# jmhb0/view_neti

Hardware: AMD Instinct MI355X
Metric: TI train steps/sec (SD-1.5 512^2 bs=4 per GPU) (higher is better)
Workload: dtype f16; 1 GPU; learnable_mode 0, sd15 shapes, 512x512 fp16, bs=4/GPU, grad_accum 1, full train step (VAE+16xCLIP+UNet fwd/bwd+AdamW); global_batch=4, parallelism=dp1, rccl_ranks=1, hipgraph=True

## Files before the change

### include/vneti.h

```cpp
#ifndef VNETI_H
#define VNETI_H
#include <stddef.h>
#include <stdint.h>

#ifdef __cplusplus
extern "C" {
#endif

#define VNETI_ABI_VERSION 1

int vneti_version(void);
int vneti_precision(void);
int vneti_last_error(char* buf, size_t n);

typedef struct vneti_gemm_desc {
  const void* A;
  const void* B;
  void* C;
  long long lda, ldb, ldc;
  int M, N, K;
  int batch;
  long long strideA, strideB, strideC;
  const float* bias;
  const void* rowadd;
  long long ld_rowadd;
  int rows_per_group;
  const void* resid;
  long long ldr;
  float alpha;
  int act;
  int out_f32;
  int conv_mode;
  int Hi, Wi, Ci, Ho, Wo, stride, pad_t, pad_l, ups;
  long long ldx;
  int tile_hint;
  void* workspace;
  long long workspace_bytes;
  int split_k;
  const void* gate_src;
  long long ld_gate;
  int gate_act;
  void* C2;
  long long ldc2;
  int act2;
  void* gn_sums;
  int gn_hw, gn_cpg, gn_groups, gn_slots;
  int geglu;
  int conv_korder;
} vneti_gemm_desc;

int vneti_gemm_f16(const vneti_gemm_desc* d, void* stream);
int vneti_gemm_select_tile(int M, int N, int batch);
int vneti_gemm_select_split(int M, int N, int K, int batch, int tile_hint, long long workspace_bytes);

int vneti_im2col3x3_small(const void* x, int x_is_f32, long long sb, long long sc, long long sy,
                          long long sx, void* out, int Bn, int C, int Hi, int Wi, int Ho, int Wo,
                          int stride, int pad_t, int pad_l, void* stream);

int vneti_conv3x3_in(const void* x, int x_is_f32, long long sb, long long sc, long long sy, long long sx,
                     const void* w_packed, const float* bias, void* out, long long ldo, int Bn, int C, int H, int W,
                     int Co, void* gn_sums, int gn_groups, int gn_slots, void* stream);

int vneti_transpose_f16(const void* in, long long ld_in, long long stride_in, void* out,
                        long long ld_out, long long stride_out, int rows, int cols, int batch,
                        void* stream);
#define VNETI_TRANSPOSE_MAX 4
typedef struct vneti_transpose_desc {
  const void* inp;
  long long ld_in, stride_in;
  void* out;
  long long ld_out, stride_out;
  int rows, cols, batch, _pad;
} vneti_transpose_desc;
int vneti_transpose_f16_multi(const vneti_transpose_desc* descs, int n, void* stream);

long long vneti_groupnorm_ws_floats(int Bn, int HW, int C, int G);
int vneti_groupnorm_fwd(const void* x, long long ldx, void* y, long long ldy, const float* gamma,
                        const float* beta, float* mean, float* rstd, float* ws, int Bn, int HW,
                        int C, int G, float eps, int silu, void* stream);
int vneti_groupnorm_fwd_sums(const void* x, long long ldx, void* y, long long ldy, const float* gamma,
                             const float* beta, const void* sums, int slots, float* mean, float* rstd,
                             int Bn, int HW, int C, int G, float eps, int silu, void* stream);
int vneti_groupnorm_fwd_2l(const void* x, long long ldx, void* y, long long ldy, const float* gamma,
                           const float* beta, void* sums, int slots, float* mean, float* rstd, int Bn, int HW,
// ... 181 lines not shown
```

### view_neti_amd/csrc/gemm8.hip

```cpp
#include <type_traits>

#include "common.h"
#include "gemm_args.h"

namespace {

constexpr int BM = 256, NT = 512;
constexpr int HALF_BYTES = 128 * 128;
constexpr int GN_IMG = 5;

#define VN_WAIT_VM(n) asm volatile("s_waitcnt vmcnt(" #n ")" ::: "memory")
#define VN_WAIT_LGKM0() asm volatile("s_waitcnt lgkmcnt(0)" ::: "memory")

template <int BN, int EPI, bool CONV, bool HALO = false>
__global__ __launch_bounds__(NT) void gemm8_kernel(GemmArgs g) {
  static_assert(BN == 256 || BN == 128, "tile width");
  static_assert(!HALO || (BN == 128 && CONV), "the halo-patch loop exists for the 256x128 convolution tile");
  constexpr int PATCH_STRIDE = 41 * 1024;
  constexpr bool H42 = HALO && BN == 128;
  constexpr int NJB = BN / 128;
  constexpr int HB_BYTES = (BN / 2) * 128;
  constexpr int HB_DMA = BN / 128;
  constexpr int NBUF = BN == 256 ? 2 : 3;
  constexpr int BUF_BYTES = 2 * HALF_BYTES + 2 * HB_BYTES;
  constexpr int CS_LD = BN + 8;
  constexpr int CS_BYTES = BM * CS_LD * 2;
  constexpr int LOOP_BYTES = HALO ? 2 * PATCH_STRIDE + 3 * 2 * HB_BYTES : NBUF * BUF_BYTES;
  constexpr int LDS_BYTES = CS_BYTES > LOOP_BYTES ? CS_BYTES : LOOP_BYTES;
  constexpr int GN_NG = BN / 4 + 2;
  const half_t* const e_gate = EPI == 2 ? g.gate_src : nullptr;
  half_t* const e_C2 = EPI == 2 ? g.C2 : nullptr;
  const int e_geglu = EPI == 2 ? g.geglu : 0;
  const int e_act = EPI == 2 ? g.act : 0;
  float* const e_gn_sums = EPI >= 1 ? g.gn_sums : nullptr;
  const half_t* const e_rowadd = EPI >= 1 ? g.rowadd : nullptr;
  const int e_conv = CONV ? g.conv_mode : 0;
  constexpr int GN_BYTES = EPI == 0 ? 0 : GN_IMG * GN_NG * 4 * 8;
  __shared__ __attribute__((aligned(16))) char smem[LDS_BYTES + GN_BYTES];

  const int tid = threadIdx.x;
  const int lane = tid & 63;
  const int wave = __builtin_amdgcn_readfirstlane(tid >> 6);
  const int wr = wave >> 2, wc = wave & 3;

  int nblk = g.tiles_m * g.tiles_n;
  int bid = blockIdx.x;
  {
    int q = nblk >> 3, r = nblk & 7, xcd = bid & 7, idx = bid >> 3;
    bid = (xcd < r ? xcd * (q + 1) : r * (q + 1) + (xcd - r) * q) + idx;
  }
  const int tile_m = bid / g.tiles_n;
  const int tile_n = bid - tile_m * g.tiles_n;
  const int m0 = tile_m * BM;
  const int n0 = tile_n * BN;
  const int bz = blockIdx.y;
  const int kz = blockIdx.z;
  int hb = 0, hty = 0, htx = 0, row0 = m0;
  if constexpr (HALO) {
    const int tpr = g.Wo >> 4, tpi = (g.Ho >> 4) * tpr;
    hb = tile_m / tpi;
    const int rem = tile_m - hb * tpi;
    hty = rem / tpr;
    htx = rem - hty * tpr;
    row0 = (hb * g.Ho + hty * 16) * g.Wo + htx * 16;
  }
  auto rowmem = [&](const int r) { return HALO ? row0 + (r >> 4) * g.Wo + (r & 15) : m0 + r; };

  const half_t* Ab = g.A + (long long)bz * g.strideA;
  const half_t* Bb = g.B + (long long)bz * g.strideB;
  const __amdgpu_buffer_rsrc_t rsA = vn_make_rsrc(Ab, g.a_bytes);
  const __amdgpu_buffer_rsrc_t rsB = vn_make_rsrc(Bb, g.b_bytes);

  const int lrow = tid >> 3;
  const int gchunk = (tid & 7) ^ ((lrow >> 1) & 7);
  const float rcp_hw = CONV ? 1.0f / (float)(g.Ho * g.Wo) : 0.f, rcp_wo = CONV ? 1.0f / (float)g.Wo : 0.f;
  int a_base[4];
  uint32_t a_mask[4];
#pragma unroll
  for (int r = 0; r < (HALO ? 0 : 4); ++r) {
// ... 719 lines not shown
      const vn_u64* src = gacc + 4 * i;
      if ((src[0] | src[1] | src[2] | src[3]) == 0) continue;
      const int img = gn_img0 + i / GN_NG, grp = gn_g0t + i % GN_NG;
      vn_u64* dst = reinterpret_cast<vn_u64*>(e_gn_sums) + (((long long)img * g.gn_slots + slot) * g.gn_G + grp) * 4;
#pragma unroll
      for (int w = 0; w < 4; ++w) atomicAdd(dst + w, src[w]);
    }
  }
}

inline int epilogue_level8(const GemmArgs& g) {
  if (g.gate_src || g.C2 || g.geglu || g.act) return 2;
  return (g.gn_sums || g.rowadd) ? 1 : 0;
}

}

int vneti_launch_gemm8(void* gemm_args, int bn, int halo, hipStream_t st) {
  GemmArgs& g = *reinterpret_cast<GemmArgs*>(gemm_args);
  if (g.out_f32 || (g.conv_mode && (g.ups || (g.conv_mode == 2 && g.stride == 2))) ||
      (g.M >= (1 << 24) && (g.conv_mode || g.rowadd || g.gn_sums)))
    return VNETI_EUNSUP;
  if (halo && (bn != 128 || g.conv_mode < 1 || g.conv_mode > 2 || g.stride != 1 || g.pad_t != 1 || g.pad_l != 1 || g.Hi != g.Ho ||
               g.Wi != g.Wo || (g.Ho & 15) || (g.Wo & 15) || (g.Ci & 63) || g.K != 9 * g.Ci || !g.korder ||
               g.batch != 1 || g.M != (g.M / (g.Ho * g.Wo)) * g.Ho * g.Wo))
    return VNETI_EUNSUP;
  if (halo && g.ksplit > 1) {
    const int nchunk = g.Ci / 64, cps = cdiv(nchunk, g.ksplit);
    g.kt_per_split = 9 * cps;
    g.ksplit = cdiv(nchunk, cps);
  }
  g.tiles_m = cdiv(g.M, BM);
  g.tiles_n = cdiv(g.N, bn);
  const dim3 grid(g.tiles_m * g.tiles_n, g.batch, g.ksplit), block(NT);
  const int epi = epilogue_level8(g);
#define VN_GO(E, C)                                                                        \
  do {                                                                                     \
    if (bn == 256) hipLaunchKernelGGL((gemm8_kernel<256, E, C>), grid, block, 0, st, g);   \
    else hipLaunchKernelGGL((gemm8_kernel<128, E, C>), grid, block, 0, st, g);             \
  } while (0)
#define VN_GO_HALO(E) hipLaunchKernelGGL((gemm8_kernel<128, E, true, true>), grid, block, 0, st, g)
  if (halo) {
    if (epi == 2) VN_GO_HALO(2); else if (epi == 1) VN_GO_HALO(1); else VN_GO_HALO(0);
  } else if (g.conv_mode) {
    if (epi == 2) VN_GO(2, true); else if (epi == 1) VN_GO(1, true); else VN_GO(0, true);
  } else {
    if (epi == 2) VN_GO(2, false); else if (epi == 1) VN_GO(1, false); else VN_GO(0, false);
  }
#undef VN_GO
#undef VN_GO_HALO
  return vneti_check_launch("gemm8_kernel");
}
```

### view_neti_amd/csrc/gemm_args.h

```cpp
#pragma once
#include "common.h"

namespace {

struct GemmArgs {
  const half_t* A;
  const half_t* B;
  void* C;
  const float* bias;
  const half_t* rowadd;
  const void* resid;
  float* ws;
  const half_t* gate_src;
  half_t* C2;
  long long ld_gate, ldc2;
  int gate_act, act2;
  float* gn_sums;
  int gn_hw, gn_cpg, gn_G, gn_slots;
  int geglu;
  long long lda, ldb, ldc, ld_rowadd, ldr;
  long long strideA, strideB, strideC;
  uint32_t a_bytes, b_bytes;
  int M, N, K;
  int rows_per_group;
  float alpha;
  int act;
  int out_f32;
  int batch, ksplit, kt_per_split;
  int conv_mode;
  int Hi, Wi, Ci, Ho, Wo, stride, pad_t, pad_l, ups;
  int ldx2;
  int korder;
  int tiles_m, tiles_n;
};

__device__ __forceinline__ float apply_act(float v, int act) {
  switch (act) {
    case 1: return vn_silu(v);
    case 2: return vn_quick_gelu(v);
    case 3: return vn_gelu_erf(v);
    default: return v;
  }
}
__device__ __forceinline__ float act_grad(float f, int act) {
  if (act == 2) {
    float s = vn_sigmoid(1.702f * f);
    return s * (1.f + 1.702f * f * (1.f - s));
  } else if (act == 3) {
    return vn_gelu_erf_grad(f);
  }
  float s = vn_sigmoid(f);
  return s * (1.f + f * (1.f - s));
}

__device__ __forceinline__ int lds_off(int row, int chunk) {
  return row * 128 + ((chunk ^ ((row >> 1) & 7)) << 4);
}

__device__ __forceinline__ void dma16(__amdgpu_buffer_rsrc_t rs, char* lds_dst, uint32_t off) {
#if defined(__HIP_DEVICE_COMPILE__)
  __builtin_amdgcn_raw_ptr_buffer_load_lds(rs, (__attribute__((address_space(3))) void*)lds_dst, 16, off, 0, 0, 0);
#else
  (void)rs; (void)lds_dst; (void)off;
#endif
}

}

int vneti_launch_gemm8(void* gemm_args, int bn, int halo, hipStream_t st);
```

### view_neti_amd/csrc/gemm_conv.hip

```cpp
#include "common.h"
#include "gemm_args.h"
#include "../../include/vneti.h"

namespace {

template <int BM, int BN, int WM, int WN, bool F32OUT, bool DMA, int NSTG = 2, int EPI = 2, bool CONV = true>
__global__ __launch_bounds__((BM / WM) * (BN / WN) * 64) void gemm_kernel(
    const half_t* pA, const half_t* pB, uint32_t p_a_bytes, uint32_t p_b_bytes, int p_lda, int p_ldb, int pM, int pN, int pK,
    int p_tiles_m, int p_tiles_n, int p_split_conv , const GemmArgs gfull) {
  GemmArgs g = gfull;
  g.A = pA;
  g.B = pB;
  g.a_bytes = p_a_bytes;
  g.b_bytes = p_b_bytes;
  g.lda = p_lda;
  g.ldb = p_ldb;
  g.M = pM;
  g.N = pN;
  g.K = pK;
  g.tiles_m = p_tiles_m;
  g.tiles_n = p_tiles_n;
  g.kt_per_split = p_split_conv & 0xffff;
  g.ksplit = (p_split_conv >> 16) & 0xff;
  g.conv_mode = p_split_conv >> 24;
  static_assert(NSTG == 2 || ((NSTG == 3 || NSTG == 4) && DMA), "the LDS rings are LDS-DMA only");
  const half_t* const e_gate = EPI == 2 ? g.gate_src : nullptr;
  half_t* const e_C2 = EPI == 2 ? g.C2 : nullptr;
  const int e_geglu = EPI == 2 ? g.geglu : 0;
  const int e_act = EPI == 2 ? g.act : 0;
  float* const e_gn_sums = EPI >= 1 ? g.gn_sums : nullptr;
  const half_t* const e_rowadd = EPI >= 1 ? g.rowadd : nullptr;
  const int e_conv = CONV ? g.conv_mode : 0;
  constexpr int NWM = BM / WM, NWN = BN / WN;
  constexpr int NT = NWM * NWN * 64;
  constexpr int RSTEP = NT / 8;
  constexpr int A_IT = BM / RSTEP, B_IT = BN / RSTEP;
  constexpr int STAGE_BYTES = (BM + BN) * 128;
  constexpr int CS_LD = F32OUT ? (BN + 4) : (BN + 8);
  constexpr int CS_BYTES = BM * CS_LD * (F32OUT ? 4 : 2);
  constexpr int LDS_BYTES = (NSTG * STAGE_BYTES > CS_BYTES) ? NSTG * STAGE_BYTES : CS_BYTES;
  constexpr int GN_IMG = 5, GN_NG = BN / 4 + 2;
  constexpr int GN_BYTES = (F32OUT || EPI == 0) ? 0 : GN_IMG * GN_NG * 4 * 8;
  __shared__ __attribute__((aligned(16))) char smem[LDS_BYTES + GN_BYTES];

  const int tid = threadIdx.x;
  const int lane = tid & 63;
  const int wave = __builtin_amdgcn_readfirstlane(tid >> 6);
  const int wm0 = (wave / NWN) * WM;
  const int wn0 = (wave % NWN) * WN;

  int nblk = g.tiles_m * g.tiles_n;
  int bid = blockIdx.x;
  {
    int q = nblk >> 3, r = nblk & 7, xcd = bid & 7, idx = bid >> 3;
    bid = (xcd < r ? xcd * (q + 1) : r * (q + 1) + (xcd - r) * q) + idx;
  }
  const int tile_m = bid / g.tiles_n;
  const int tile_n = bid - tile_m * g.tiles_n;
  const int m0 = tile_m * BM;
  const int n0 = tile_n * BN;
  const int bz = blockIdx.y;
  const int kz = blockIdx.z;

  const half_t* Ab = g.A + (long long)bz * g.strideA;
  const half_t* Bb = g.B + (long long)bz * g.strideB;
  __amdgpu_buffer_rsrc_t rsA = vn_make_rsrc(Ab, g.a_bytes);
  __amdgpu_buffer_rsrc_t rsB = vn_make_rsrc(Bb, g.b_bytes);

  const int lrow = tid >> 3;
  const int gchunk = DMA ? ((tid & 7) ^ ((lrow >> 1) & 7)) : (tid & 7);

  const float rcp_hw = CONV ? __builtin_amdgcn_rcpf((float)(g.Ho * g.Wo)) : 0.f, rcp_wo = CONV ? __builtin_amdgcn_rcpf((float)g.Wo) : 0.f;
  int a_off[A_IT];
  int a_py[A_IT], a_px[A_IT], a_bh[A_IT];
#pragma unroll
  for (int i = 0; i < A_IT; ++i) {
    int m = m0 + lrow + RSTEP * i;
    bool ok = m < g.M;
    if (e_conv == 0) {
      a_off[i] = ok ? (int)((long long)m * g.lda * 2) + gchunk * 16 : -1;
      a_py[i] = a_px[i] = a_bh[i] = 0;
    } else {
      int rem, ox;
      const int b = vn_divmod(m, g.Ho * g.Wo, rcp_hw, rem);
      const int oy = vn_divmod(rem, g.Wo, rcp_wo, ox);
// ... 535 lines not shown
  for (int z = 0; z < g.ksplit; ++z) {
    const float* p = p0 + z * zstride;
    for (int e = 0; e < ne; ++e) v[e] += p[e];
  }
  for (int e = 0; e < ne; ++e) {
    float x = v[e] * g.alpha;
    if (g.bias) x += g.bias[c + e];
    x = apply_act(x, g.act);
    if (g.out_f32) {
      if (g.resid) x += reinterpret_cast<const float*>(g.resid)[(long long)bz * g.strideC + (long long)m * g.ldr + c + e];
      reinterpret_cast<float*>(g.C)[(long long)bz * g.strideC + (long long)m * g.ldc + c + e] = x;
    } else {
      x = (float)(half_t)x;
      if (g.rowadd) x = (float)(half_t)(x + (float)g.rowadd[(long long)(m / g.rows_per_group) * g.ld_rowadd + c + e]);
      if (g.resid)
        x = (float)(half_t)(x + (float)reinterpret_cast<const half_t*>(g.resid)[(long long)bz * g.strideC + (long long)m * g.ldr + c + e]);
      if (g.gate_src) x = (float)(half_t)(x * act_grad((float)g.gate_src[(long long)m * g.ld_gate + c + e], g.gate_act));
      reinterpret_cast<half_t*>(g.C)[(long long)bz * g.strideC + (long long)m * g.ldc + c + e] = (half_t)x;
      if (g.C2) g.C2[(long long)m * g.ldc2 + c + e] = (half_t)apply_act((float)(half_t)x, g.act2);
    }
  }
}

inline int epilogue_level(const GemmArgs& g) {
  if (g.gate_src || g.C2 || g.geglu || g.act) return 2;
  return (g.gn_sums || g.rowadd) ? 1 : 0;
}

template <int BM, int BN, int WM, int WN, bool F32OUT, bool DMA, int NSTG>
void launch_variant(const GemmArgs& g, dim3 grid, hipStream_t st) {
  const dim3 block((BM / WM) * (BN / WN) * 64);
#define VN_GO(E, C)                                                                                                        \
  hipLaunchKernelGGL((gemm_kernel<BM, BN, WM, WN, F32OUT, DMA, NSTG, E, C>), grid, block, 0, st, g.A, g.B, g.a_bytes, g.b_bytes, \
                     (int)g.lda, (int)g.ldb, g.M, g.N, g.K, g.tiles_m, g.tiles_n, g.kt_per_split | (g.ksplit << 16) | (g.conv_mode << 24), g)
  if constexpr (F32OUT) {
    if (g.conv_mode) { if (g.act) VN_GO(2, true); else VN_GO(0, true); }
    else { if (g.act) VN_GO(2, false); else VN_GO(0, false); }
  } else {
    const int epi = epilogue_level(g);
    if (g.conv_mode) { if (epi == 2) VN_GO(2, true); else if (epi == 1) VN_GO(1, true); else VN_GO(0, true); }
    else { if (epi == 2) VN_GO(2, false); else if (epi == 1) VN_GO(1, false); else VN_GO(0, false); }
  }
#undef VN_GO
}

inline void launch_reduce(const GemmArgs& g, hipStream_t st) {
  if (g.ksplit > 1) {
    long long total = (long long)g.batch * g.M * ((g.N + 3) / 4);
    hipLaunchKernelGGL(splitk_reduce_kernel, dim3((unsigned)cdivl(total, 256)), dim3(256), 0, st, g.ws, g.C, g.bias, g.resid,
                       g.rowadd, g.M, g.N, g.batch, g.ksplit, (int)g.ldc, (int)g.ldr, g);
  }
}

template <int BM, int BN, int WM, int WN, bool DMA>
int launch_cfg(GemmArgs& g, bool f32out, hipStream_t st) {
  g.tiles_m = cdiv(g.M, BM);
  g.tiles_n = cdiv(g.N, BN);
  dim3 grid(g.tiles_m * g.tiles_n, g.batch, g.ksplit);
  if (f32out) launch_variant<BM, BN, WM, WN, true, DMA, 2>(g, grid, st);
  else launch_variant<BM, BN, WM, WN, false, DMA, 2>(g, grid, st);
  launch_reduce(g, st);
  return vneti_check_launch("gemm_kernel");
}

template <int BM, int BN, int WM, int WN, int NSTG = 3>
int launch_cfg_ring(GemmArgs& g, bool f32out, hipStream_t st) {
  g.tiles_m = cdiv(g.M, BM);
  g.tiles_n = cdiv(g.N, BN);
  dim3 grid(g.tiles_m * g.tiles_n, g.batch, g.ksplit);
  if (f32out) launch_variant<BM, BN, WM, WN, true, true, NSTG>(g, grid, st);
  else launch_variant<BM, BN, WM, WN, false, true, NSTG>(g, grid, st);
  launch_reduce(g, st);
  return vneti_check_launch("gemm_kernel");
}

template <int BM, int BN, int WM, int WN, bool DMA>
int launch_cfg_f16(GemmArgs& g, hipStream_t st) {
  g.tiles_m = cdiv(g.M, BM);
  g.tiles_n = cdiv(g.N, BN);
  dim3 grid(g.tiles_m * g.tiles_n, g.batch, g.ksplit);
  launch_variant<BM, BN, WM, WN, false, DMA, 2>(g, grid, st);
  launch_reduce(g, st);
  return vneti_check_launch("gemm_kernel");
}

struct TileDims {
  int bm, bn;
};
constexpr int kMaxTile = 18;
constexpr TileDims kTiles[kMaxTile + 1] = {{0, 0},     {128, 128}, {128, 64},  {64, 64},  {256, 128}, {256, 256}, {256, 128}, {256, 128},
                                          {256, 128}, {128, 128}, {128, 128}, {128, 64},  {64, 64},   {128, 128}, {128, 64},  {64, 64},
                                          {256, 256}, {256, 128}, {256, 128}};

int select_tile(int M, int N, int batch) {
  long long t256 = (long long)cdiv(M, 256) * cdiv(N, 128) * batch;
  long long t128 = (long long)cdiv(M, 128) * cdiv(N, 128) * batch;
  long long t12864 = (long long)cdiv(M, 128) * cdiv(N, 64) * batch;
  if (N <= 64) return (M >= 2048) ? 2 : 3;
  (void)t256;
  if (t128 >= 384) return 1;
  if (t12864 >= 384) return 2;
  return 3;
}

int select_ksplit(int M, int N, int K, int batch, int tile, long long ws_floats) {
  if (ws_floats <= 0) return 1;
  const int nk = K / 64;
  long long tiles = (long long)cdiv(M, kTiles[tile].bm) * cdiv(N, kTiles[tile].bn) * batch;
  if (tiles >= 256 || nk < 16) return 1;
  int s = (int)(512 / tiles);
  if (s > nk / 8) s = nk / 8;
  if (s > 16) s = 16;
  while (s > 1 && (long long)s * batch * M * N > ws_floats) --s;
  return s < 2 ? 1 : s;
}

}

extern "C" int vneti_gemm_select_tile(int M, int N, int batch) { return select_tile(M, N, batch > 0 ? batch : 1); }

extern "C" int vneti_gemm_select_split(int M, int N, int K, int batch, int tile_hint, long long workspace_bytes) {
  if (batch <= 0) batch = 1;
  int cfg = tile_hint >= 100 ? tile_hint - 100 : tile_hint;
  if (cfg == 0) cfg = select_tile(M, N, batch);
  if (cfg < 1 || cfg > kMaxTile || K % 64 != 0) return -1;
  int ks = select_ksplit(M, N, K, batch, cfg, workspace_bytes / 4);
  const int nk = K / 64;
  if (ks > nk) ks = nk;
  if (ks < 1) ks = 1;
  return cdiv(nk, cdiv(nk, ks));
}

extern "C" int vneti_gemm_f16(const vneti_gemm_desc* d, void* stream) {
  VN_REQUIRE(d != nullptr, "gemm: null descriptor");
  VN_REQUIRE(d->A && d->B && d->C, "gemm: null operand pointer");
  VN_REQUIRE(d->M > 0 && d->N > 0 && d->K > 0, "gemm: bad shape M=%d N=%d K=%d", d->M, d->N, d->K);
  VN_REQUIRE(d->K % 64 == 0, "gemm: K=%d must be a multiple of 64", d->K);
  VN_REQUIRE(d->ldb % 8 == 0, "gemm: ldb=%lld must be a multiple of 8", d->ldb);
  int batch = d->batch > 0 ? d->batch : 1;
  GemmArgs g;
  memset(&g, 0, sizeof(g));
  g.A = (const half_t*)d->A;
  g.B = (const half_t*)d->B;
  g.C = d->C;
  g.bias = d->bias;
  g.rowadd = (const half_t*)d->rowadd;
  g.resid = d->resid;
  g.gate_src = (const half_t*)d->gate_src;
  g.ld_gate = d->ld_gate;
  g.gate_act = d->gate_act;
  g.C2 = (half_t*)d->C2;
  g.ldc2 = d->ldc2;
  g.act2 = d->act2;
  g.gn_sums = (float*)d->gn_sums;
  g.gn_hw = d->gn_hw;
  g.gn_cpg = d->gn_cpg;
  g.gn_G = d->gn_groups;
  g.gn_slots = d->gn_slots;
  g.geglu = d->geglu;
  g.lda = d->lda;
  g.ldb = d->ldb;
  g.ldc = d->ldc;
  g.ld_rowadd = d->ld_rowadd;
  g.ldr = d->ldr;
  g.strideA = d->strideA;
  g.strideB = d->strideB;
  g.strideC = d->strideC;
  g.M = d->M;
  g.N = d->N;
  g.K = d->K;
  g.batch = batch;
  g.rows_per_group = d->rows_per_group > 0 ? d->rows_per_group : 1;
  g.alpha = d->alpha;
  g.act = d->act;
  g.out_f32 = d->out_f32 ? 1 : 0;
  g.conv_mode = d->conv_mode;
  long long a_bytes;
  if (d->conv_mode == 0) {
    VN_REQUIRE(d->lda % 8 == 0, "gemm: lda=%lld must be a multiple of 8", d->lda);
    a_bytes = ((long long)(d->M - 1) * d->lda + d->K) * 2;
  } else {
    VN_REQUIRE(d->conv_mode == 1 || d->conv_mode == 2, "gemm: bad conv_mode %d", d->conv_mode);
    VN_REQUIRE(d->Ci > 0 && d->Ci % 64 == 0, "conv: Ci=%d must be a multiple of 64", d->Ci);
    VN_REQUIRE(d->K == 9 * d->Ci, "conv: K=%d must equal 9*Ci=%d", d->K, 9 * d->Ci);
    VN_REQUIRE(d->stride == 1 || d->stride == 2, "conv: stride %d unsupported", d->stride);
    VN_REQUIRE(d->Ho > 0 && d->Wo > 0 && d->M % (d->Ho * d->Wo) == 0, "conv: M=%d not a multiple of Ho*Wo", d->M);
    VN_REQUIRE(d->ldx % 8 == 0, "conv: ldx must be a multiple of 8");
    VN_REQUIRE(!(d->ups && d->conv_mode != 1), "conv: fused upsample only in forward gather mode");
    VN_REQUIRE(!(d->ups && d->stride != 1), "conv: fused upsample needs stride 1");
    g.Hi = d->Hi;
    g.Wi = d->Wi;
    g.Ci = d->Ci;
    g.Ho = d->Ho;
    g.Wo = d->Wo;
    g.stride = d->stride;
    g.pad_t = d->pad_t;
    g.pad_l = d->pad_l;
    g.ups = d->ups;
    g.ldx2 = (int)(d->ldx * 2);
    VN_REQUIRE(!d->conv_korder || d->Ci % 64 == 0, "conv: conv_korder=1 needs Ci=%d to be a multiple of 64", d->Ci);
    g.korder = d->conv_korder ? 1 : 0;
    long long nb = d->M / (d->Ho * d->Wo);
    a_bytes = nb * d->Hi * d->Wi * d->ldx * 2;
  }
  long long b_bytes = ((long long)(d->N - 1) * d->ldb + d->K) * 2;
  VN_REQUIRE(a_bytes < 0x7fffffffLL && b_bytes < 0x7fffffffLL, "gemm: operand larger than 2 GiB");
  g.a_bytes = (uint32_t)a_bytes;
  g.b_bytes = (uint32_t)b_bytes;
  if (!d->out_f32) {
// ... 105 lines not shown
```

### view_neti_amd/engine/schedule.py

```python
from __future__ import annotations

from functools import partial
from typing import Dict, List

import torch

from .. import lib, ops, packing


class T:

    __slots__ = ("v", "g", "gw", "rows", "cols", "children", "need_grad", "producer")

    def __init__(self, v, g=None, need_grad=True):
        self.v = v
        self.g = g
        self.gw = False
        self.rows, self.cols = v.shape
        self.children: List["T"] = []
        self.need_grad = need_grad
        self.producer = None


def rup(x, m):
# ... 411 lines not shown


def _timing_switches(dev, reps):
    import os
    cold = None if os.environ.get("VNETI_AUTOTUNE_HOT") else torch.empty(160 * 2 ** 20, dtype=torch.float32, device=dev)
    return (cold, reps, int(os.environ.get("VNETI_AUTOTUNE_REPS", "9")),
            bool(int(os.environ.get("VNETI_AUTOTUNE_WARM_A", "1"))))


def _time_call(call, act, cold, reps, cold_reps, warm_a):
    call()
    call()

    def timed(n):
        s, e = torch.cuda.Event(enable_timing=True), torch.cuda.Event(enable_timing=True)
        s.record()
        for _ in range(n):
            call()
        e.record()
        e.synchronize()
        return s.elapsed_time(e)

    if cold is None:
        return timed(reps)
    ts = []
    for _ in range(cold_reps):
        cold.fill_(0)
        if warm_a:
            act.add_(0)
        ts.append(timed(1))
    return sorted(ts)[len(ts) // 2]


def picks_to_json(cache: Dict) -> Dict:
    return {repr(k): [int(x) for x in v] for k, v in cache.items()}


def picks_from_json(data: Dict) -> Dict:
    import ast
    return {ast.literal_eval(k): tuple(int(x) for x in v) for k, v in data.items()}


def export_picks() -> Dict:
    from ..roofline import kernel_tree_sha
    return {"kernel_tree_sha": kernel_tree_sha(), "picks": picks_to_json(Schedule._tile_cache)}


def preload_picks(data: Dict) -> bool:
    from ..roofline import kernel_tree_sha
    if data.get("kernel_tree_sha") != kernel_tree_sha():
        return False
    Schedule._tile_cache.update(picks_from_json(data["picks"]))
    return True
```

### view_neti_amd/engine/step.py

```python
from __future__ import annotations

from functools import partial
from typing import Dict, List, Optional

import torch

from .. import ops
from .. import sd_config as sc
from .graphs import capture_graphs
from .text import MapperState, TextEngine
from .unet import UNetEngine
from .vae import VAEEncoderEngine


def alphas_cumprod(cfg: sc.DDPMConfig) -> torch.Tensor:
    betas = torch.linspace(cfg.beta_start ** 0.5, cfg.beta_end ** 0.5, cfg.num_train_timesteps,
                           dtype=torch.float32) ** 2
    return torch.cumprod(1.0 - betas, dim=0)


class TrainStepEngine:
    def __init__(self, cfg: sc.SDConfig, unet_w: Dict, vae_w: Dict, clip_w: Dict, batch: int, height: int,
                 width: int, mapper_object: Dict[str, torch.Tensor], w_enc_object: torch.Tensor,
                 norm_scale_object: Optional[float], alpha_object: float = 0.2,
# ... 61 lines not shown
        mo = MapperState(self.params[:n_all_obj],
                         w_enc_object.to(device).float().contiguous() if legacy_pe_object is None else None,
                         norm_scale_object, alpha_object, hidden=hidden_object, enc_dim=enc_dim_object,
                         unconstrained=unconstrained_object,
                         nested_dropout_prob=nested_dropout_prob, slot=self.obj_slot if multi else None,
                         slot_stride=self.n_obj if multi else 0,
                         legacy_w_pe=(legacy_pe_object.to(device).float().contiguous()
                                      if legacy_pe_object is not None else None),
                         output_bypass=output_bypass_object)
        mv, gv = None, None
        if mapper_view is not None:
            if flat_v is not None:
                pv, gv = self.params[n_all_obj:], self.grads[n_all_obj:]
            else:
                pv = flatten_mapper_state(mapper_view).to(device)
            mv = MapperState(pv, w_enc_view.to(device).float().contiguous(), norm_scale_view, alpha_view,
                             unconstrained=unconstrained_view,
                             nested_dropout_prob=nested_dropout_prob if flat_v is not None else 0.0,
                             output_bypass=output_bypass_view)
        self.grad_accum = grad_accum
        self.hyper = torch.tensor([lr, betas[0], betas[1], adam_eps, weight_decay, float(world_size * grad_accum)],
                                  dtype=torch.float32, device=device)
        self.scaler = torch.tensor([loss_scale, 0.0, 0.0], dtype=torch.float32, device=device)
        self.opt_step = torch.zeros(1, dtype=torch.int32, device=device)
        self.loss_sum = torch.zeros(1, dtype=torch.float32, device=device)
        self.ac = alphas_cumprod(cfg.ddpm).to(device)
        from ..parallel import shared_picks
        with shared_picks():
            self.unet = UNetEngine(cfg.unet, unet_w, batch, self.h, self.w, cfg.clip.max_positions, device, need_backward)
            self.vae = VAEEncoderEngine(cfg.vae, vae_w, batch, height, width, device)
            self.text = TextEngine(cfg.clip, clip_w, cfg.unet.n_cross_layers, batch, self.unet.timesteps, self.unet.ctx_k,
                                   self.unet.ctx_v, self.unet.dctx_k, self.unet.dctx_v, mo, self.grads[:n_all_obj], mv,
                                   gv, n_view_params, train_view, device, need_backward, rng_state=self.rng_state)
        self.timesteps = self.unet.timesteps
        self.pixel_values = self.vae.x_in
        shape = (batch, Lc, self.h, self.w)
        self.eps = torch.zeros(shape, dtype=torch.float32, device=device)
        self.noise = torch.zeros(shape, dtype=torch.float32, device=device)
        self.latents = torch.zeros(shape, dtype=torch.float32, device=device)
        self.target = torch.zeros(shape, dtype=torch.float32, device=device)
        self.n_cache = int(moment_cache_images)
        if self.n_cache:
            hw2 = self.h * self.w
            self.mcache = torch.zeros(self.n_cache, hw2, 2 * Lc, dtype=self.vae.moments.dtype, device=device)
            self.img_idx = torch.zeros(batch, dtype=torch.int64, device=device)
            self._cached_images = set()
            self._batch_cached = False
            self._batch_images = ()
        self.graph_a_c = self.graph_acc_c = None
        self.eval_out = torch.zeros(batch, dtype=torch.float32, device=device)
        self.eval_ws = torch.zeros(ops.mse_loss_per_sample_ws_floats(batch, self.h * self.w), dtype=torch.float32,
                                   device=device)
        self.graph_eval = None
        from .staging import HostStager
        self.stager = HostStager()
        self.need_backward = need_backward
        self.overlap = overlap
        self.side = torch.cuda.Stream() if overlap else None
        self.graph_a = self.graph_b = self.graph_acc = None
        self.exchange_in_graph = False
        self._reduce_stage = None
        self.last_reduce_bytes = 0
        self.micro = 0
        self._eval_batch = False
        self.n_loss = batch * Lc * self.h * self.w

# ... 313 lines not shown
```

### view_neti_amd/ops.py

```python
from __future__ import annotations

import ctypes as C

import torch

from . import lib as _l

ACT_NONE, ACT_SILU, ACT_QUICK_GELU, ACT_GELU = 0, 1, 2, 3


def stream() -> int:
    return torch.cuda.current_stream().cuda_stream


def _p(t):
    return None if t is None else t.data_ptr()


def _ld(t):
    if t is None:
        return 0
    assert t.stride(-1) == 1, "last dim must be contiguous"
    return t.stride(-2) if t.dim() >= 2 else t.shape[-1]


_default_ws = None


def set_default_gemm_workspace(t):
    global _default_ws
    _default_ws = t


def gemm(A, B, out, *, bias=None, rowadd=None, rows_per_group=1, resid=None, alpha=1.0, act=0,
         tile_hint=0, batch=0, strideA=0, strideB=0, strideC=0, M=None, N=None, K=None, conv=None,
         lda=None, ldc=None, workspace=None, split_k=0, gate=None, gate_act=0, out2=None, act2=0,
         gn_sums=None, gn_hw=0, gn_groups=0, gn_slots=0, geglu=0):
    d = _l.GemmDesc()
    d.A, d.B, d.C = _p(A), _p(B), _p(out)
    d.ldb = _ld(B)
    d.ldc = ldc if ldc is not None else _ld(out)
    d.N = N if N is not None else B.shape[-2]
    d.K = K if K is not None else B.shape[-1]
    if conv is None:
        d.M = M if M is not None else A.shape[-2]
        d.lda = lda if lda is not None else _ld(A)
        d.conv_mode = 0
    else:
        d.M = M
        d.lda = 0
        d.conv_mode = conv["mode"]
        for k in ("Hi", "Wi", "Ci", "Ho", "Wo", "stride", "pad_t", "pad_l", "ups", "ldx"):
            setattr(d, k, int(conv.get(k, 0)))
        d.conv_korder = int(conv.get("korder", 0))
    d.batch = batch
    d.strideA, d.strideB, d.strideC = strideA, strideB, strideC
    d.bias = _p(bias)
    d.rowadd = _p(rowadd)
    d.ld_rowadd = _ld(rowadd) if rowadd is not None else 0
    d.rows_per_group = rows_per_group
    d.resid = _p(resid)
    d.ldr = _ld(resid) if resid is not None else 0
    d.alpha = alpha
    d.act = act
    d.out_f32 = 1 if out.dtype == torch.float32 else 0
    d.tile_hint = tile_hint
    if gate is not None:
        d.gate_src, d.ld_gate, d.gate_act = _p(gate), _ld(gate), gate_act
    if out2 is not None:
        d.C2, d.ldc2, d.act2 = _p(out2), _ld(out2), act2
    if gn_sums is not None:
        d.gn_sums, d.gn_hw, d.gn_groups, d.gn_slots = _p(gn_sums), gn_hw, gn_groups, gn_slots
        d.gn_cpg = d.N // gn_groups
    d.geglu = geglu
    ws = workspace if workspace is not None else _default_ws
    if ws is not None:
        d.workspace = ws.data_ptr()
        d.workspace_bytes = ws.numel() * ws.element_size()
    d.split_k = split_k if ws is not None else 1
    _l.call("gemm_f16", C.byref(d), stream())


def im2col3x3_small(x, out, Bn, Cc, Hi, Wi, Ho, Wo, stride, pad_t, pad_l, strides):
    sb, sc, sy, sx = strides
    _l.call("im2col3x3_small", _p(x), 1 if x.dtype == torch.float32 else 0, sb, sc, sy, sx, _p(out),
            Bn, Cc, Hi, Wi, Ho, Wo, stride, pad_t, pad_l, stream())


def conv3x3_in(x, w_packed, bias, out, Bn, Cc, H, W, strides, gn_sums=None, gn_hw=0, gn_groups=0, gn_slots=0):
    sb, sc, sy, sx = strides
    assert gn_sums is None or gn_hw == H * W
    _l.call("conv3x3_in", _p(x), 1 if x.dtype == torch.float32 else 0, sb, sc, sy, sx, _p(w_packed), _p(bias), _p(out),
            _ld(out), Bn, Cc, H, W, w_packed.shape[0], _p(gn_sums), gn_groups, gn_slots, stream())


def transpose(inp, out, rows, cols, batch, ld_in, stride_in, ld_out, stride_out):
    _l.call("transpose_f16", _p(inp), ld_in, stride_in, _p(out), ld_out, stride_out, rows, cols, batch, stream())


def transpose_multi(items):
    arr = (_l.TransposeDesc * len(items))()
    for d, (inp, out, rows, cols, batch, ld_in, stride_in, ld_out, stride_out) in zip(arr, items):
        d.inp, d.ld_in, d.stride_in = _p(inp), ld_in, stride_in
        d.out, d.ld_out, d.stride_out = _p(out), ld_out, stride_out
        d.rows, d.cols, d.batch = rows, cols, batch
    _l.call("transpose_f16_multi", arr, len(items), stream())


def groupnorm_ws_floats(Bn, HW, Cc, G):
    n = _l.query("groupnorm_ws_floats", Bn, HW, Cc, G)
    if n < 0:
        raise RuntimeError(f"groupnorm: unsupported shape {(Bn, HW, Cc, G)}")
    return n
# ... 387 lines not shown
```

Measured before the change: 38.94 steps/s.

## Prefetch next GEMM's weights into cache using extra workgroups in current GEMM

Adds extra workgroups to each GEMM launch. They read the next scheduled GEMM's weight tensor, discard the data and exit, with the goal of warming the last-level (MALL/L2) cache. A scheduler pass links each GEMM to its successor across the forward and backward lists. It only does so when the traffic in between fits in the cache budget and the next weights are at most 5 MiB. The feature is on by default through an environment variable. The cost is extra memory bandwidth and a few CUs taken from the main GEMM tiles, and it relies on packing the prefetch workgroup count into the high bits of p_split_conv.

```diff
diff --git a/include/vneti.h b/include/vneti.h
--- a/include/vneti.h
+++ b/include/vneti.h
@@ -47,9 +47,12 @@
   int gn_hw, gn_cpg, gn_groups, gn_slots;
   int geglu;
   int conv_korder;
+  const void* next_w;
+  long long next_w_bytes;
 } vneti_gemm_desc;
 
 int vneti_gemm_f16(const vneti_gemm_desc* d, void* stream);
+int vneti_gemm_last_grid(int* xyz);
 int vneti_gemm_select_tile(int M, int N, int batch);
 int vneti_gemm_select_split(int M, int N, int K, int batch, int tile_hint, long long workspace_bytes);
 
diff --git a/view_neti_amd/csrc/gemm8.hip b/view_neti_amd/csrc/gemm8.hip
--- a/view_neti_amd/csrc/gemm8.hip
+++ b/view_neti_amd/csrc/gemm8.hip
@@ -13,7 +13,8 @@
 #define VN_WAIT_LGKM0() asm volatile("s_waitcnt lgkmcnt(0)" ::: "memory")
 
 template <int BN, int EPI, bool CONV, bool HALO = false>
-__global__ __launch_bounds__(NT) void gemm8_kernel(GemmArgs g) {
+__global__ __launch_bounds__(NT) void gemm8_kernel(
+    const int pf_wgs, GemmArgs g) {
   static_assert(BN == 256 || BN == 128, "tile width");
   static_assert(!HALO || (BN == 128 && CONV), "the halo-patch loop exists for the 256x128 convolution tile");
   constexpr int PATCH_STRIDE = 41 * 1024;
@@ -38,13 +39,19 @@
   constexpr int GN_BYTES = EPI == 0 ? 0 : GN_IMG * GN_NG * 4 * 8;
   __shared__ __attribute__((aligned(16))) char smem[LDS_BYTES + GN_BYTES];
 
+  if ((int)blockIdx.x < pf_wgs) {
+    vn_prefetch_share(g.next_w, g.next_w_bytes, (int)(blockIdx.x + pf_wgs * (blockIdx.y + gridDim.y * blockIdx.z)),
+                      (int)(pf_wgs * gridDim.y * gridDim.z), (int)threadIdx.x, NT);
+    return;
+  }
+
   const int tid = threadIdx.x;
   const int lane = tid & 63;
   const int wave = __builtin_amdgcn_readfirstlane(tid >> 6);
   const int wr = wave >> 2, wc = wave & 3;
 
   int nblk = g.tiles_m * g.tiles_n;
-  int bid = blockIdx.x;
+  int bid = (int)blockIdx.x - pf_wgs;
   {
     int q = nblk >> 3, r = nblk & 7, xcd = bid & 7, idx = bid >> 3;
     bid = (xcd < r ? xcd * (q + 1) : r * (q + 1) + (xcd - r) * q) + idx;
@@ -830,14 +837,16 @@
   }
   g.tiles_m = cdiv(g.M, BM);
   g.tiles_n = cdiv(g.N, bn);
-  const dim3 grid(g.tiles_m * g.tiles_n, g.batch, g.ksplit), block(NT);
+  g.pf_wgs = vn_prefetch_wgs(g.next_w_bytes, g.batch * g.ksplit, g.tiles_m * g.tiles_n);
+  const dim3 grid(g.pf_wgs + g.tiles_m * g.tiles_n, g.batch, g.ksplit), block(NT);
+  vn_note_gemm_grid(grid.x, grid.y, grid.z);
   const int epi = epilogue_level8(g);
 #define VN_GO(E, C)                                                                        \
   do {                                                                                     \
-    if (bn == 256) hipLaunchKernelGGL((gemm8_kernel<256, E, C>), grid, block, 0, st, g);   \
-    else hipLaunchKernelGGL((gemm8_kernel<128, E, C>), grid, block, 0, st, g);             \
+    if (bn == 256) hipLaunchKernelGGL((gemm8_kernel<256, E, C>), grid, block, 0, st, g.pf_wgs, g);   \
+    else hipLaunchKernelGGL((gemm8_kernel<128, E, C>), grid, block, 0, st, g.pf_wgs, g);             \
   } while (0)
-#define VN_GO_HALO(E) hipLaunchKernelGGL((gemm8_kernel<128, E, true, true>), grid, block, 0, st, g)
+#define VN_GO_HALO(E) hipLaunchKernelGGL((gemm8_kernel<128, E, true, true>), grid, block, 0, st, g.pf_wgs, g)
   if (halo) {
     if (epi == 2) VN_GO_HALO(2); else if (epi == 1) VN_GO_HALO(1); else VN_GO_HALO(0);
   } else if (g.conv_mode) {
diff --git a/view_neti_amd/csrc/gemm_args.h b/view_neti_amd/csrc/gemm_args.h
--- a/view_neti_amd/csrc/gemm_args.h
+++ b/view_neti_amd/csrc/gemm_args.h
@@ -32,7 +32,25 @@
   int ldx2;
   int korder;
   int tiles_m, tiles_n;
+  int pf_wgs;
+  const void* next_w;
+  long long next_w_bytes;
 };
+
+constexpr long long VN_PF_SHARE_BYTES = 128 * 1024;
+constexpr int VN_PF_MAX_WGS = 32;
+constexpr int VN_PF_INFLIGHT = 8;
+constexpr int VN_PF_CUS = 256;
+static_assert(VN_PF_MAX_WGS < 64, "the workgroup count travels in six bits of p_split_conv");
+
+inline int vn_prefetch_wgs(long long bytes, int slices, int tiles_per_slice) {
+  if (bytes <= 0) return 0;
+  const long long total = (long long)tiles_per_slice * slices;
+  const long long room = (total < VN_PF_CUS ? VN_PF_CUS - total : total / 16) / slices;
+  long long want = cdivl(cdivl(bytes, VN_PF_SHARE_BYTES), slices);
+  if (want > room) want = room;
+  return (int)(want > VN_PF_MAX_WGS ? VN_PF_MAX_WGS : want);
+}
 
 __device__ __forceinline__ float apply_act(float v, int act) {
   switch (act) {
@@ -65,6 +83,27 @@
 #endif
 }
 
+__device__ __forceinline__ void vn_prefetch_share(const void* p, long long bytes, int share, int nshares, int tid, int nt) {
+  const __amdgpu_buffer_rsrc_t rs = vn_make_rsrc(p, (uint32_t)bytes);
+  const uint32_t nchunk = (uint32_t)((bytes + 15) >> 4);
+  const uint32_t per = (nchunk + (uint32_t)nshares - 1) / (uint32_t)nshares;
+  const uint32_t begin = (uint32_t)share * per;
+  const uint32_t end = begin + per < nchunk ? begin + per : nchunk;
+  uint32_t fold = 0;
+  for (uint32_t c = begin + (uint32_t)tid; c < end; c += (uint32_t)nt * VN_PF_INFLIGHT) {
+    u32x4 v[VN_PF_INFLIGHT];
+#pragma unroll
+    for (int u = 0; u < VN_PF_INFLIGHT; ++u) {
+      const uint32_t cu = c + (uint32_t)(u * nt);
+      v[u] = vn_buf_load16(rs, cu < end ? cu << 4 : VN_OOB);
+    }
+#pragma unroll
+    for (int u = 0; u < VN_PF_INFLIGHT; ++u) fold |= v[u][0] ^ v[u][1] ^ v[u][2] ^ v[u][3];
+  }
+  asm volatile("" ::"v"(fold));
+}
+
 }
 
 int vneti_launch_gemm8(void* gemm_args, int bn, int halo, hipStream_t st);
+void vn_note_gemm_grid(unsigned x, unsigned y, unsigned z);
diff --git a/view_neti_amd/csrc/gemm_conv.hip b/view_neti_amd/csrc/gemm_conv.hip
--- a/view_neti_amd/csrc/gemm_conv.hip
+++ b/view_neti_amd/csrc/gemm_conv.hip
@@ -7,7 +7,14 @@
 template <int BM, int BN, int WM, int WN, bool F32OUT, bool DMA, int NSTG = 2, int EPI = 2, bool CONV = true>
 __global__ __launch_bounds__((BM / WM) * (BN / WN) * 64) void gemm_kernel(
     const half_t* pA, const half_t* pB, uint32_t p_a_bytes, uint32_t p_b_bytes, int p_lda, int p_ldb, int pM, int pN, int pK,
-    int p_tiles_m, int p_tiles_n, int p_split_conv , const GemmArgs gfull) {
+    int p_tiles_m, int p_tiles_n, int p_split_conv ,
+    const GemmArgs gfull) {
+  const int pf_wgs = (int)((uint32_t)p_split_conv >> 26);
+  if ((int)blockIdx.x < pf_wgs) {
+    vn_prefetch_share(gfull.next_w, gfull.next_w_bytes, (int)(blockIdx.x + pf_wgs * (blockIdx.y + gridDim.y * blockIdx.z)),
+                      (int)(pf_wgs * gridDim.y * gridDim.z), (int)threadIdx.x, (BM / WM) * (BN / WN) * 64);
+    return;
+  }
   GemmArgs g = gfull;
   g.A = pA;
   g.B = pB;
@@ -22,7 +29,7 @@
   g.tiles_n = p_tiles_n;
   g.kt_per_split = p_split_conv & 0xffff;
   g.ksplit = (p_split_conv >> 16) & 0xff;
-  g.conv_mode = p_split_conv >> 24;
+  g.conv_mode = (p_split_conv >> 24) & 3;
   static_assert(NSTG == 2 || ((NSTG == 3 || NSTG == 4) && DMA), "the LDS rings are LDS-DMA only");
   const half_t* const e_gate = EPI == 2 ? g.gate_src : nullptr;
   half_t* const e_C2 = EPI == 2 ? g.C2 : nullptr;
@@ -50,7 +57,7 @@
   const int wn0 = (wave % NWN) * WN;
 
   int nblk = g.tiles_m * g.tiles_n;
-  int bid = blockIdx.x;
+  int bid = (int)blockIdx.x - pf_wgs;
   {
     int q = nblk >> 3, r = nblk & 7, xcd = bid & 7, idx = bid >> 3;
     bid = (xcd < r ? xcd * (q + 1) : r * (q + 1) + (xcd - r) * q) + idx;
@@ -652,7 +659,10 @@
   const dim3 block((BM / WM) * (BN / WN) * 64);
 #define VN_GO(E, C)                                                                                                        \
   hipLaunchKernelGGL((gemm_kernel<BM, BN, WM, WN, F32OUT, DMA, NSTG, E, C>), grid, block, 0, st, g.A, g.B, g.a_bytes, g.b_bytes, \
-                     (int)g.lda, (int)g.ldb, g.M, g.N, g.K, g.tiles_m, g.tiles_n, g.kt_per_split | (g.ksplit << 16) | (g.conv_mode << 24), g)
+                     (int)g.lda, (int)g.ldb, g.M, g.N, g.K, g.tiles_m, g.tiles_n,        \
+                     (int)((uint32_t)g.kt_per_split | ((uint32_t)g.ksplit << 16) | ((uint32_t)g.conv_mode << 24) |              \
+                           ((uint32_t)g.pf_wgs << 26)),                                                                           \
+                     g)
   if constexpr (F32OUT) {
     if (g.conv_mode) { if (g.act) VN_GO(2, true); else VN_GO(0, true); }
     else { if (g.act) VN_GO(2, false); else VN_GO(0, false); }
@@ -676,7 +686,9 @@
 int launch_cfg(GemmArgs& g, bool f32out, hipStream_t st) {
   g.tiles_m = cdiv(g.M, BM);
   g.tiles_n = cdiv(g.N, BN);
-  dim3 grid(g.tiles_m * g.tiles_n, g.batch, g.ksplit);
+  g.pf_wgs = vn_prefetch_wgs(g.next_w_bytes, g.batch * g.ksplit, g.tiles_m * g.tiles_n);
+  dim3 grid(g.pf_wgs + g.tiles_m * g.tiles_n, g.batch, g.ksplit);
+  vn_note_gemm_grid(grid.x, grid.y, grid.z);
   if (f32out) launch_variant<BM, BN, WM, WN, true, DMA, 2>(g, grid, st);
   else launch_variant<BM, BN, WM, WN, false, DMA, 2>(g, grid, st);
   launch_reduce(g, st);
@@ -687,7 +699,9 @@
 int launch_cfg_ring(GemmArgs& g, bool f32out, hipStream_t st) {
   g.tiles_m = cdiv(g.M, BM);
   g.tiles_n = cdiv(g.N, BN);
-  dim3 grid(g.tiles_m * g.tiles_n, g.batch, g.ksplit);
+  g.pf_wgs = vn_prefetch_wgs(g.next_w_bytes, g.batch * g.ksplit, g.tiles_m * g.tiles_n);
+  dim3 grid(g.pf_wgs + g.tiles_m * g.tiles_n, g.batch, g.ksplit);
+  vn_note_gemm_grid(grid.x, grid.y, grid.z);
   if (f32out) launch_variant<BM, BN, WM, WN, true, true, NSTG>(g, grid, st);
   else launch_variant<BM, BN, WM, WN, false, true, NSTG>(g, grid, st);
   launch_reduce(g, st);
@@ -698,7 +712,9 @@
 int launch_cfg_f16(GemmArgs& g, hipStream_t st) {
   g.tiles_m = cdiv(g.M, BM);
   g.tiles_n = cdiv(g.N, BN);
-  dim3 grid(g.tiles_m * g.tiles_n, g.batch, g.ksplit);
+  g.pf_wgs = vn_prefetch_wgs(g.next_w_bytes, g.batch * g.ksplit, g.tiles_m * g.tiles_n);
+  dim3 grid(g.pf_wgs + g.tiles_m * g.tiles_n, g.batch, g.ksplit);
+  vn_note_gemm_grid(grid.x, grid.y, grid.z);
   launch_variant<BM, BN, WM, WN, false, DMA, 2>(g, grid, st);
   launch_reduce(g, st);
   return vneti_check_launch("gemm_kernel");
@@ -735,6 +751,18 @@
   return s < 2 ? 1 : s;
 }
 
+}
+
+static thread_local int t_last_grid[3] = {0, 0, 0};
+void vn_note_gemm_grid(unsigned x, unsigned y, unsigned z) {
+  t_last_grid[0] = (int)x;
+  t_last_grid[1] = (int)y;
+  t_last_grid[2] = (int)z;
+}
+extern "C" int vneti_gemm_last_grid(int* xyz) {
+  VN_REQUIRE(xyz != nullptr, "gemm_last_grid: null output");
+  for (int i = 0; i < 3; ++i) xyz[i] = t_last_grid[i];
+  return VNETI_OK;
 }
 
 extern "C" int vneti_gemm_select_tile(int M, int N, int batch) { return select_tile(M, N, batch > 0 ? batch : 1); }
@@ -795,6 +823,10 @@
   g.act = d->act;
   g.out_f32 = d->out_f32 ? 1 : 0;
   g.conv_mode = d->conv_mode;
+  VN_REQUIRE(d->next_w_bytes >= 0 && d->next_w_bytes < 0x7fffffffLL, "gemm: next_w_bytes=%lld out of range", d->next_w_bytes);
+  VN_REQUIRE(d->next_w_bytes == 0 || d->next_w != nullptr, "gemm: next_w_bytes without next_w");
+  g.next_w = d->next_w;
+  g.next_w_bytes = d->next_w ? d->next_w_bytes : 0;
   long long a_bytes;
   if (d->conv_mode == 0) {
     VN_REQUIRE(d->lda % 8 == 0, "gemm: lda=%lld must be a multiple of 8", d->lda);
diff --git a/view_neti_amd/engine/schedule.py b/view_neti_amd/engine/schedule.py
--- a/view_neti_amd/engine/schedule.py
+++ b/view_neti_amd/engine/schedule.py
@@ -467,6 +467,54 @@
     return sorted(ts)[len(ts) // 2]
 
 
+MALL_BYTES = 256 * 2 ** 20
+PREFETCH_MAX_BYTES = 5 * 2 ** 20
+PREFETCH_MAX_BETWEEN = MALL_BYTES
+PREFETCH_MIN_BYTES = 0
+WEIGHT_PREFETCH_DEFAULT = "1"
+
+
+def weight_prefetch_enabled() -> bool:
+    import os
+    return os.environ.get("VNETI_WEIGHT_PREFETCH", WEIGHT_PREFETCH_DEFAULT) != "0"
+
+
+def _tensor_bytes(f, skip=()):
+    kw = getattr(f, "keywords", None) or {}
+    args = list(getattr(f, "args", ())) + [v for k, v in kw.items() if k not in skip]
+    return sum(t.numel() * t.element_size() for t in args if isinstance(t, torch.Tensor))
+
+
+def _weight_range(f):
+    Bm, kw = f.args[1], f.keywords
+    N, K = kw.get("N") or Bm.shape[-2], kw.get("K") or Bm.shape[-1]
+    batch = kw.get("batch") or 1
+    elems = (batch - 1) * (kw.get("strideB") or 0) + (N - 1) * Bm.stride(-2) + K
+    return Bm.data_ptr(), elems * Bm.element_size()
+
+
+def wire_weight_prefetch(lists, wrap: bool = True) -> int:
+    seq = [(lst, i) for lst in lists for i in range(len(lst))]
+    at = [k for k, (lst, i) in enumerate(seq) if getattr(lst[i], "func", None) is ops.gemm]
+    if len(at) < 2:
+        return 0
+    n = 0
+    for a, b in zip(at, at[1:] + (at[:1] if wrap else [])):
+        lst, i = seq[a]
+        f, nxt = lst[i], seq[b][0][seq[b][1]]
+        between = range(a + 1, b) if b > a else list(range(a + 1, len(seq))) + list(range(0, b))
+        moved = _tensor_bytes(f, skip=("workspace",)) - _weight_range(f)[1] + \
+            sum(_tensor_bytes(seq[k][0][seq[k][1]]) for k in between)
+        if moved > PREFETCH_MAX_BETWEEN:
+            continue
+        addr, nbytes = _weight_range(nxt)
+        if nbytes < PREFETCH_MIN_BYTES or nbytes > PREFETCH_MAX_BYTES:
+            continue
+        lst[i] = partial(ops.gemm, *f.args, **dict(f.keywords, prefetch=(addr, nbytes)))
+        n += 1
+    return n
+
+
 def picks_to_json(cache: Dict) -> Dict:
     return {repr(k): [int(x) for x in v] for k, v in cache.items()}
 
diff --git a/view_neti_amd/engine/step.py b/view_neti_amd/engine/step.py
--- a/view_neti_amd/engine/step.py
+++ b/view_neti_amd/engine/step.py
@@ -117,6 +117,12 @@
             self.text = TextEngine(cfg.clip, clip_w, cfg.unet.n_cross_layers, batch, self.unet.timesteps, self.unet.ctx_k,
                                    self.unet.ctx_v, self.unet.dctx_k, self.unet.dctx_v, mo, self.grads[:n_all_obj], mv,
                                    gv, n_view_params, train_view, device, need_backward, rng_state=self.rng_state)
+        from .schedule import weight_prefetch_enabled, wire_weight_prefetch
+        self.n_weight_prefetch = 0
+        if weight_prefetch_enabled():
+            self.n_weight_prefetch = wire_weight_prefetch(
+                [self.vae.fwd, self.text.fwd, self.unet.fwd_pre, self.unet.fwd] +
+                ([self.unet.bwd, self.text.bwd] if need_backward else []))
         self.timesteps = self.unet.timesteps
         self.pixel_values = self.vae.x_in
         shape = (batch, Lc, self.h, self.w)
diff --git a/view_neti_amd/ops.py b/view_neti_amd/ops.py
--- a/view_neti_amd/ops.py
+++ b/view_neti_amd/ops.py
@@ -35,7 +35,7 @@
 def gemm(A, B, out, *, bias=None, rowadd=None, rows_per_group=1, resid=None, alpha=1.0, act=0,
          tile_hint=0, batch=0, strideA=0, strideB=0, strideC=0, M=None, N=None, K=None, conv=None,
          lda=None, ldc=None, workspace=None, split_k=0, gate=None, gate_act=0, out2=None, act2=0,
-         gn_sums=None, gn_hw=0, gn_groups=0, gn_slots=0, geglu=0):
+         gn_sums=None, gn_hw=0, gn_groups=0, gn_slots=0, geglu=0, prefetch=None):
     d = _l.GemmDesc()
     d.A, d.B, d.C = _p(A), _p(B), _p(out)
     d.ldb = _ld(B)
@@ -78,7 +78,16 @@
         d.workspace = ws.data_ptr()
         d.workspace_bytes = ws.numel() * ws.element_size()
     d.split_k = split_k if ws is not None else 1
+    if prefetch is not None:
+        d.next_w, d.next_w_bytes = prefetch if isinstance(prefetch, tuple) else \
+            (prefetch.data_ptr(), prefetch.numel() * prefetch.element_size())
     _l.call("gemm_f16", C.byref(d), stream())
+
+
+def gemm_last_grid():
+    xyz = (C.c_int * 3)()
+    _l.call("gemm_last_grid", xyz)
+    return tuple(xyz)
 
 
 def im2col3x3_small(x, out, Bn, Cc, Hi, Wi, Ho, Wo, stride, pad_t, pad_l, strides):
```

Measured after the change: 38.79 steps/s. About the same (-0.4%).
